# DaehwanKimLab/tophat

Hardware: AMD Instinct MI355X
Metric: paired reads/sec through segment_juncs+long_spanning_reads; junctions.bed diff=0 (higher is better)
Workload: dtype u64

## Files before the change

### tophat_amd/csrc/thj_core.h

```cpp
#pragma once
#include <stdint.h>

#if defined(__HIPCC__)
#define THJ_HD __host__ __device__ __forceinline__
#else
#define THJ_HD inline
#endif

#if defined(THJ_EXP) && defined(__HIPCC__)
static __device__ int thj_exp_flags;
#define THJ_EXPF(b) (thj_exp_flags & (b))
#else
#define THJ_EXPF(b) 0
#endif

namespace thj {

typedef unsigned long long u64;

THJ_HD int popc(u64 x) { return __builtin_popcountll(x); }
THJ_HD int popc32(uint32_t x) { return __builtin_popcount(x); }
THJ_HD int ctz(u64 x) { return __builtin_ctzll(x); }
THJ_HD int clz(u64 x) { return __builtin_clzll(x); }
THJ_HD u64 lowmask(int n) { return n >= 64 ? ~0ull : ((1ull << n) - 1ull); }
// ... 564 lines not shown
template <int NS>
THJ_HD bool read_is_trivial_flat(const Params& p, const ReadView& v) {
    const int nseg = v.nseg;
    const uint32_t first = v.so[0];
    if (v.so[nseg] == first) return true;
    bool single = true;
#pragma unroll
    for (int s = 0; s < NS; ++s) single = single && (s >= nseg || v.so[s + 1] - v.so[s] == 1u);
    if (!single) return false;
    Hit h[NS];
#pragma unroll
    for (int s = 0; s < NS; ++s) if (s < nseg) h[s] = v.hits[first + s];
    const Hit h0 = h[0];
    const bool anti = hit_anti(h0);
    if (nseg == 1) return hit_end(h0) || v.n_mate == 0;
    const int L = p.segment_length;
    bool ok = true;
    Hit prev = h0;
#pragma unroll
    for (int s = 1; s < NS; ++s) {
        if (s < nseg) {
            const Hit c = h[s];
            ok = ok && c.ref_id == h0.ref_id && hit_anti(c) == anti;
            ok = ok && (anti ? c.right == prev.left : prev.right == c.left);
            if (s + 1 < nseg) {
                const int start = (s - 1) * L;
                const int plen = v.rl - start < 2 * L ? v.rl - start : 2 * L;
                const int apparent = anti ? prev.right - c.left : c.right - prev.left;
                ok = ok && start <= v.rl && apparent == plen;
            }
            prev = c;
        }
    }
    if (!ok) return false;
    const int dist = anti ? h0.left - prev.right : prev.left - h0.right;
    if (dist >= p.min_segment_intron && dist < p.max_segment_intron) return true;
    return v.n_mate == 0;
}

THJ_HD bool read_is_trivial(const Params& p, const ReadView& v) {
    if (v.nseg < 1) return true;
    if (v.nseg <= 4) return read_is_trivial_flat<4>(p, v);
    const uint32_t first = v.so[0];
    if (v.so[v.nseg] == first) return true;
    for (int s = 0; s < v.nseg; ++s) if (v.so[s + 1] - v.so[s] != 1u) return false;
    const Hit h0 = v.hits[first];
    const bool anti = hit_anti(h0);
    if (v.nseg == 1) return hit_end(h0) || v.n_mate == 0;
    const int L = p.segment_length;
    Hit prev = h0;
    for (int s = 1; s < v.nseg; ++s) {
        const Hit h = v.hits[first + s];
        if (h.ref_id != h0.ref_id || hit_anti(h) != anti) return false;
        if (!((anti && h.right == prev.left) || (!anti && prev.right == h.left))) return false;
        if (s + 1 < v.nseg) {
            const int start = (s - 1) * L;
            if (start > v.rl) return false;
            const int plen = v.rl - start < 2 * L ? v.rl - start : 2 * L;
            const int apparent = anti ? prev.right - h.left : h.right - prev.left;
            if (apparent != plen) return false;
        }
        prev = h;
    }
    const int dist = anti ? h0.left - prev.right : prev.left - h0.right;
    if (dist >= p.min_segment_intron && dist < p.max_segment_intron) return true;
    return v.n_mate == 0;
}

THJ_HD uint32_t task_window_word(bool anti, int start, int slen) { return (anti ? 1u << 9 : 0u) | ((uint32_t)(start & 511) << 10) | ((uint32_t)(slen & 127) << 19); }
THJ_HD uint32_t task_indel_word(bool anti, bool is_del, int i, int plen) {
    return (1u << 8) | (anti ? 1u << 9 : 0u) | (is_del ? 1u << 10 : 0u) | ((uint32_t)(i & 15) << 11) | ((uint32_t)(plen & 255) << 15);
}
THJ_HD bool task_is_indel(uint32_t a) { return (a & (1u << 8)) != 0; }
THJ_HD bool task_anti(uint32_t a) { return ((a >> 9) & 1u) != 0; }
THJ_HD bool task_is_del(uint32_t a) { return ((a >> 10) & 1u) != 0; }
THJ_HD int task_indel_i(uint32_t a) { return (int)((a >> 11) & 15u); }
THJ_HD int task_indel_plen(uint32_t a) { return (int)((a >> 15) & 255u); }
THJ_HD int task_window_start(uint32_t a) { return (int)((a >> 10) & 511u); }
THJ_HD int task_window_slen(uint32_t a) { return (int)((a >> 19) & 127u); }

struct FlatResult { bool rescue; int size; int n_windows, n_indels; };

template <int NS, class Emit>
THJ_HD FlatResult flat_read(const Params& p, int nseg, const uint32_t (&so)[NS + 1], const Hit (&h)[NS], int rl, int n_mate, Emit& emit) {
    FlatResult res{false, 0, 0, 0};
    const int L = p.segment_length;
    uint32_t present = 0;
#pragma unroll
    for (int s = 0; s < NS; ++s) if (s < nseg && so[s + 1] != so[s]) present |= 1u << s;
    bool go = true;
#pragma unroll
    for (int i = 0; i + 2 < NS; ++i) {
        const int start = i * L;
        go = go && i + 2 < nseg && ((present >> i) & 3u) == 3u && start <= rl;
        const int plen = rl - start < 2 * L ? rl - start : 2 * L;
        const Hit lh = h[i], rh = h[i + 1];
        const bool anti = hit_anti(lh);
        const int apparent = anti ? lh.right - rh.left : rh.right - lh.left;
        const int disc = apparent - plen;
        const bool is_del = disc > 0 && disc <= p.max_deletion_length;
        const bool is_ins = disc < 0 && disc >= -p.max_insertion_length;
        const bool ok = go && lh.ref_id == rh.ref_id && anti == hit_anti(rh) && (is_del || is_ins);
        emit.task(ok, task_indel_word(anti, is_del, i, plen), anti ? so[i + 1] : so[i], anti ? so[i] : so[i + 1], 0u);
        res.n_indels += ok ? 1 : 0;
    }
    int last = 0;
    Hit hl = h[0];
#pragma unroll
    for (int s = 1; s < NS; ++s) if ((present >> s) & 1u) { last = s; hl = h[s]; }
    res.size = last + 1;
    bool run = nseg > 0;
    if (last == 0) run = run && (present & 1u) && !hit_end(h[0]);
    bool check_partner = true;
    if (last != 0 && (present & 1u) && h[0].ref_id == hl.ref_id && hit_anti(h[0]) == hit_anti(hl)) {
        const int dist = hit_anti(h[0]) ? h[0].left - hl.right : hl.left - h[0].right;
        if (dist >= p.min_segment_intron && dist < p.max_segment_intron) check_partner = false;
    }
    res.rescue = run && check_partner && n_mate > 0;
    bool en = run && !res.rescue;
    if (p.bowtie2 && present != 0 && 1 > p.max_seg_multihits) en = false;
#pragma unroll
    for (int s = 0; s + 1 < NS; ++s) {
        const bool has = en && s != last && ((present >> s) & 1u);
        const Hit bh = h[s];
        const bool banti = hit_anti(bh);
        const Hit rh = h[s + 1];
        const bool c1 = ((present >> (s + 1)) & 1u) && banti == hit_anti(rh) && bh.ref_id == rh.ref_id;
        const bool abut = banti ? rh.right == bh.left : bh.right == rh.left;
        const int d1 = banti ? bh.left - rh.right : rh.left - bh.right;
        const bool found = c1 && abut;
        const bool drs = c1 && !abut && d1 >= p.min_segment_intron && d1 < p.max_segment_intron;
        bool rrs = false;
        Hit d = rh;
        if (s + 2 < NS) {
            const Hit rrh = h[s + 2];
            const bool c2 = ((present >> (s + 2)) & 1u) && banti == hit_anti(rrh) && bh.ref_id == rrh.ref_id;
            const int d2 = banti ? bh.left - rrh.right : rrh.left - bh.right;
            rrs = !found && c2 && d2 >= p.min_segment_intron + L && d2 < p.max_segment_intron + L;
            if (rrs) d = rrh;
        }
        const int start = (s + 1) * L - 8;
        int slen = rrs ? L + 16 : 16;
        if (slen > rl - start) slen = rl - start;
        int32_t wl, wr;
        if (!banti) { wl = bh.right - 8; if (wl < 0) wl = 0; wr = d.left + 8; }
        else { wl = d.right - 8; wr = bh.left + 8; }
        const bool ok = has && !found && (drs || rrs) && start >= 0 && slen >= 0;
        emit.task(ok, task_window_word(banti, start, slen), bh.ref_id, (uint32_t)wl, (uint32_t)wr);
        res.n_windows += ok ? 1 : 0;
    }
    return res;
}

enum { SLOT_UNSCANNED = -3 };
template <int MAXM, class Emit>
THJ_HD int flat_rescue(const Params& p, bool has0, const Hit& bh, int size, int rl, const Hit (&mh)[MAXM], int n_mate,
                       const int32_t (&sc)[2 * MAXM], Emit& emit, int& n_windows) {
    const int L = p.segment_length;
    int cl = L - p.segment_mismatches - 3;
    if (cl > 15) cl = 15;
    const bool banti = hit_anti(bh);
    bool alive = has0;
    int pairs = 0, n_pseudo = 0;
    int32_t pl[2 * MAXM];
    bool pv[2 * MAXM];
#pragma unroll
    for (int m = 0; m < MAXM; ++m) {
        const bool compat = alive && m < n_mate && bh.ref_id == mh[m].ref_id && banti != hit_anti(mh[m]);
        const int32_t f = compat ? sc[2 * m] : SLOT_NONE, rv = compat ? sc[2 * m + 1] : SLOT_NONE;
        if (compat && f == SLOT_BREAK) alive = false;
        pairs += (compat && f != SLOT_BREAK && f != SLOT_UNSCANNED) ? 1 : 0;
        pv[2 * m] = compat && alive && f >= 0; pl[2 * m] = f;
        pv[2 * m + 1] = compat && alive && rv >= 0; pl[2 * m + 1] = rv;
        n_pseudo += (pv[2 * m] ? 1 : 0) + (pv[2 * m + 1] ? 1 : 0);
    }
    bool en = has0 && (size == 2 || size == 3);
    if (p.bowtie2 && (1 > p.max_seg_multihits || n_pseudo > p.max_seg_multihits)) en = false;
    const bool far = size == 3;
    const int lo = p.min_segment_intron + (far ? L : 0), hi = p.max_segment_intron + (far ? L : 0);
    bool found = false, inr[2 * MAXM];
    int n = 0;
#pragma unroll
    for (int k = 0; k < 2 * MAXM; ++k) {
        const bool panti = (k & 1) != 0;
        const bool c = pv[k] && banti == panti;
        const int32_t pleft = pl[k], pright = pl[k] + cl;
        const bool abut = banti ? pright == bh.left : bh.right == pleft;
        if (c && abut && !far) found = true;
        const int dist = banti ? bh.left - pright : pleft - bh.right;
        inr[k] = c && dist >= lo && dist < hi;
        n += inr[k] ? 1 : 0;
    }
    const int start = L - 8;
    int slen = far ? L + 16 : 16;
    if (slen > rl - start) slen = rl - start;
    const bool ok_all = en && !found && n > 0 && start >= 0 && slen >= 0;
#pragma unroll
    for (int k = 0; k < 2 * MAXM; ++k) {
        const int32_t pleft = pl[k], pright = pl[k] + cl;
        int32_t wl, wr;
        if (!banti) { wl = bh.right - 8; if (wl < 0) wl = 0; wr = pleft + 8; }
        else { wl = pright - 8; wr = bh.left + 8; }
        const bool ok = ok_all && inr[k];
        emit.task(ok, task_window_word(banti, start, slen), bh.ref_id, (uint32_t)wl, (uint32_t)wr);
        n_windows += ok ? 1 : 0;
    }
    return pairs;
}

template <class Sink>
THJ_HD void gaps_enumerate(const Params& p, const ReadView& v, Sink& sink, int first = 0, int stride = 1) {
    const int L = p.segment_length;
    if (p.bowtie2)
        for (int s = 0; s < v.size; ++s) {
            int n = (!v.rescue || s == 0) ? rv_count_raw(v, s) : rv_count(v, s);
            if (n > p.max_seg_multihits) return;
        }
    for (int s = 0; s < v.size; ++s) {
        rv_foreach_strided(v, s, first, stride, [&](const Hit& bh) {
            bool found = (s == v.size - 1);
            int n_drs = 0, n_rrs = 0;
            const bool banti = hit_anti(bh);
            if (s < v.size - 1) {
                rv_foreach(v, s + 1, [&](const Hit& rh) {
                    if (banti != hit_anti(rh) || bh.ref_id != rh.ref_id) return true;
                    if ((banti && rh.right == bh.left) || (!banti && bh.right == rh.left)) { found = true; return false; }
                    int dist = banti ? bh.left - rh.right : rh.left - bh.right;
                    if (dist >= p.min_segment_intron && dist < p.max_segment_intron) ++n_drs;
                    return true;
                });
            }
            if (!found && s < v.size - 2) {
                rv_foreach(v, s + 2, [&](const Hit& rrh) {
                    if (banti != hit_anti(rrh) || bh.ref_id != rrh.ref_id) return true;
                    int dist = banti ? bh.left - rrh.right : rrh.left - bh.right;
                    if (dist >= p.min_segment_intron + L && dist < p.max_segment_intron + L) ++n_rrs;
                    return true;
                });
            }
            if (!found && (n_drs > 0 || n_rrs > 0)) {
                const bool use_rrs = n_rrs > 0;
                const int lo = p.min_segment_intron + (use_rrs ? L : 0);
                const int hi = p.max_segment_intron + (use_rrs ? L : 0);
                const int start = (s + 1) * L - 8;
                int slen = use_rrs ? L + 16 : 16;
                if (slen > v.rl - start) slen = v.rl - start;
                if (start >= 0 && slen >= 0) {
                    rv_foreach(v, use_rrs ? s + 2 : s + 1, [&](const Hit& d) {
                        if (banti != hit_anti(d) || bh.ref_id != d.ref_id) return true;
                        int dist = banti ? bh.left - d.right : d.left - bh.right;
                        if (dist < lo || dist >= hi) return true;
                        int32_t wl, wr;
                        if (!banti) { wl = bh.right - 8; if (wl < 0) wl = 0; wr = d.left + 8; }
                        else { wl = d.right - 8; wr = bh.left + 8; }
                        sink.window(bh.ref_id, wl, wr, banti, start, slen);
                        return true;
                    });
                }
            }
        });
    }
}

template <class X>
THJ_HD Hit wave_bcast_hit(X& x, const Hit& h, int src) {
    Hit o;
    o.ref_id = x.bcast(h.ref_id, src); o.left = (int32_t)x.bcast((uint32_t)h.left, src);
    o.right = (int32_t)x.bcast((uint32_t)h.right, src); o.meta = x.bcast(h.meta, src);
    return o;
}
THJ_HD Hit wave_lane_hit(const ReadView& v, int s, int lane) {
    Hit h{0, 0, 0, 0};
    if (lane < rv_count_raw(v, s)) h = v.hits[v.so[s] + (uint32_t)lane];
    return h;
}
THJ_HD bool wave_read_fits(const ReadView& v) {
    for (int s = 0; s < v.nseg; ++s) if (rv_count_raw(v, s) > 64) return false;
    return true;
}
template <class X, class Sink>
THJ_HD bool wave_read_enumerate(X& x, const Params& p, ReadView& v, Sink& sink, bool& wants_rescue) {
    const int lane = x.lane;
    const int L = p.segment_length;
    wants_rescue = false;
    v.rescue = false;
    v.check_len = p.segment_length - p.segment_mismatches - 3;
    if (v.check_len > 15) v.check_len = 15;
    if (v.nseg == 0) return false;
    int last = v.nseg - 1;
    while (last > 0 && rv_count_raw(v, last) == 0) --last;
    v.size = last + 1;
    if (last == 0) {
        if (rv_count_raw(v, 0) == 0) return false;
        const Hit h0 = v.hits[v.so[0]];
        if (hit_end(h0)) return false;
    }
    {
        bool found = false;
        if (last != 0) {
            const Hit lh = wave_lane_hit(v, 0, lane);
            const bool have = lane < rv_count_raw(v, 0);
            const Hit D = wave_lane_hit(v, last, lane);
            const int nD = rv_count_raw(v, last);
            for (int j = 0; j < nD; ++j) {
                const Hit rh = wave_bcast_hit(x, D, j);
                if (have && lh.ref_id == rh.ref_id && hit_anti(lh) == hit_anti(rh)) {
// ... 351 lines not shown
```

### tophat_amd/csrc/thj_segjuncs.hip

```cpp
#include <hip/hip_runtime.h>
#include <hipcub/hipcub.hpp>

#include <cstdio>
#include <cstdlib>
#include <algorithm>
#include <cstring>
#include <cstddef>
#include <chrono>
#include <vector>

#include "../../include/thj.h"
#include "thj_core.h"
#include "thj_fusion_block.h"
#include "thj_internal.h"

using namespace thj;

static_assert(sizeof(thj_hit) == 16 && sizeof(Hit) == 16, "hit layout");
static_assert(sizeof(thj_params) == sizeof(Params), "params layout");




static constexpr u64 EMPTY = ~0ull;
// ... 3 lines not shown
struct Tables {
    u64* junc; u64 junc_mask;
    u64* del;  u64 del_mask;
    u64* ins_key; u64* ins_val; u64 ins_mask;
    u64* junc_list; u64* del_list; u64* ins_list;
    unsigned int* ovf;
    unsigned long long* cnt;
};

__device__ __forceinline__ u64 mix64(u64 x) {
    x ^= x >> 30; x *= 0xbf58476d1ce4e5b9ull;
    x ^= x >> 27; x *= 0x94d049bb133111ebull;
    x ^= x >> 31;
    return x;
}

__device__ __forceinline__ unsigned long long list_append_pos(unsigned long long* count) {
    const int lane = (int)(threadIdx.x & 63u);
    const unsigned long long below = lane ? (~0ull >> (64 - lane)) : 0ull;
    for (;;) {
        const unsigned long long mine_p = (unsigned long long)count;
        const unsigned long long p0 = ((unsigned long long)(uint32_t)__builtin_amdgcn_readfirstlane((int)(uint32_t)(mine_p >> 32)) << 32) |
                                      (uint32_t)__builtin_amdgcn_readfirstlane((int)(uint32_t)mine_p);
        const bool now = mine_p == p0;
        const unsigned long long grp = __ballot(now);
        if (now) {
            unsigned long long base = 0;
            if (lane == __ffsll((long long)grp) - 1) base = atomicAdd(count, (unsigned long long)__popcll(grp));
            const uint32_t lo = (uint32_t)__builtin_amdgcn_readfirstlane((int)(uint32_t)base), hi = (uint32_t)__builtin_amdgcn_readfirstlane((int)(uint32_t)(base >> 32));
            return (((unsigned long long)hi << 32) | lo) + (unsigned long long)__popcll(grp & below);
        }
    }
}

static constexpr u64 PROBE_CAP = 4096;
template <bool RESCUE = false>
__device__ __forceinline__ void set_insert(u64* tab, u64 mask, u64 key, unsigned long long* count, unsigned int* ovf, u64* list) {
    if (!RESCUE && __hip_atomic_load(ovf, __ATOMIC_RELAXED, __HIP_MEMORY_SCOPE_AGENT) != 0u) return;
    u64 h = mix64(key) & mask;
    const u64 limit = RESCUE ? mask : (mask < PROBE_CAP ? mask : PROBE_CAP);
    for (u64 probe = 0; probe <= limit; ++probe) {
        u64 cur = __hip_atomic_load(&tab[h], __ATOMIC_RELAXED, __HIP_MEMORY_SCOPE_AGENT);
        if (cur == key) return;
        if (cur == EMPTY) {
            u64 old = atomicCAS((unsigned long long*)&tab[h], EMPTY, key);
            if (old == EMPTY) { const unsigned long long pos = list_append_pos(count); if (pos <= mask) list[pos] = key; return; }
            if (old == key) return;
        }
        h = (h + 1) & mask;
    }
    atomicExch(ovf, 1u);
}

template <bool RESCUE = false>
__device__ __forceinline__ void map_insert_min(u64* keys, u64* vals, u64 mask, u64 key, u64 val,
                                               unsigned long long* count, unsigned int* ovf, u64* list) {
    if (!RESCUE && __hip_atomic_load(ovf, __ATOMIC_RELAXED, __HIP_MEMORY_SCOPE_AGENT) != 0u) return;
    u64 h = mix64(key) & mask;
    const u64 limit = RESCUE ? mask : (mask < PROBE_CAP ? mask : PROBE_CAP);
    for (u64 probe = 0; probe <= limit; ++probe) {
        u64 cur = __hip_atomic_load(&keys[h], __ATOMIC_RELAXED, __HIP_MEMORY_SCOPE_AGENT);
        if (cur == EMPTY) {
            u64 old = atomicCAS((unsigned long long*)&keys[h], EMPTY, key);
            if (old == EMPTY) { const unsigned long long pos = list_append_pos(count); if (pos <= mask) list[pos] = h; cur = key; }
            else cur = old;
        }
        if (cur == key) { atomicMin((unsigned long long*)&vals[h], val); return; }
        h = (h + 1) & mask;
    }
    atomicExch(ovf, 1u);
}

struct EventSink {
    const Genome& g;
    const Tables& t;
    __device__ __forceinline__ void junction(uint32_t ref, uint32_t l, uint32_t r, bool a) {
        set_insert(t.junc, t.junc_mask, junc_key(g, ref, l, r, a), &t.cnt[CNT_JUNC], &t.ovf[0], t.junc_list);
    }
    __device__ __forceinline__ void deletion(uint32_t ref, uint32_t l, uint32_t r) {
        set_insert(t.del, t.del_mask, junc_key(g, ref, l, r, false), &t.cnt[CNT_DEL], &t.ovf[1], t.del_list);
    }
    __device__ __forceinline__ void insertion(uint32_t ref, uint32_t l, int len, uint32_t seq, u64 prio) {
        map_insert_min(t.ins_key, t.ins_val, t.ins_mask, ins_key(g, ref, l, len), (prio << INS_SEQ_BITS) | (u64)(seq & ((1u << INS_SEQ_BITS) - 1u)),
                       &t.cnt[CNT_INS], &t.ovf[2], t.ins_list);
    }
};


struct DevBatch {
    int32_t n_reads, nseg, W, pad;
    const uint32_t* seg_off;
    const Hit* hits;
    const u64* planes;
    const uint16_t* read_len;
    const uint32_t* mate_off;
    const Hit* mate_hits;
    uint32_t ordinal_base, pad2;
};
static_assert(sizeof(DevBatch) == sizeof(thj_seg_batch), "batch layout");

__device__ __forceinline__ ReadView make_view(const DevBatch& b, int r) {
    ReadView v;
    v.hits = b.hits;
    v.so = b.seg_off + (size_t)r * b.nseg;
    v.nseg = b.nseg;
    v.W = b.W;
    v.rp = b.planes + (size_t)r * 3 * b.W;
    v.rl = b.read_len[r];
    v.mate = nullptr; v.n_mate = 0; v.slots = nullptr; v.mscan = nullptr;
    if (b.mate_off) {
        uint32_t m0 = b.mate_off[r], m1 = b.mate_off[r + 1];
        v.mate = b.mate_hits + m0;
        v.n_mate = (int)(m1 - m0);
    }
    v.size = 0; v.rescue = false; v.check_len = 0;
    return v;
}


static constexpr int TPB = 256;
static constexpr int QCAP = 512;
static constexpr int MANY_CAP = 1 << 20;
static constexpr int MANY_HITS_LDS = 256;

struct Queue {
    uint32_t* a; uint32_t* b; uint32_t* c; uint32_t* d; uint32_t* e;
    unsigned int* n;
};
struct XTasks { uint4* q; uint32_t* e; unsigned int* count; unsigned int cap; unsigned int* ovf; };

struct QueueSink {
    Queue q;
    XTasks x;
    uint32_t read;
    uint32_t hbase;
    unsigned int n_windows, n_indels;
    __device__ __forceinline__ void push(uint32_t a, uint32_t b, uint32_t c, uint32_t d) {
        unsigned int k = atomicAdd(q.n, 1u);
        if (k < (unsigned)QCAP) { q.a[k] = a; q.b[k] = b; q.c[k] = c; q.d[k] = d; q.e[k] = read; }
        else {
            const unsigned int pos = atomicAdd(x.count, 1u);
            if (pos < x.cap) { x.q[pos] = make_uint4(a, b, c, d); x.e[pos] = read; } else atomicExch(x.ovf, 1u);
        }
    }
    __device__ __forceinline__ void window(uint32_t ref, int32_t wl, int32_t wr, bool anti, int start, int slen) {
        ++n_windows;
        push(task_window_word(anti, start, slen), ref, (uint32_t)wl, (uint32_t)wr);
    }
    __device__ __forceinline__ void indel(int i, uint32_t lidx, uint32_t ridx, int li, int ri, bool anti, int plen, bool is_del) {
        ++n_indels;
        push(task_indel_word(anti, is_del, i, plen), lidx + hbase, ridx + hbase, (uint32_t)li | ((uint32_t)ri << 16));
    }
};
__device__ __forceinline__ void flush_tasks(const Queue& q, const XTasks& x, unsigned int* s_base, unsigned int* full_rounds) {
    __syncthreads();
    const unsigned int have = *q.n, n = have < (unsigned)QCAP ? have : (unsigned)QCAP;
    if (have == 0) return;
    if (threadIdx.x == 0) { *s_base = atomicAdd(x.count, n); if (have > (unsigned)QCAP) atomicAdd(full_rounds, 1u); }
    __syncthreads();
    const unsigned int base = *s_base;
    for (unsigned int k = threadIdx.x; k < n; k += blockDim.x) {
        const unsigned int pos = base + k;
        if (pos < x.cap) { x.q[pos] = make_uint4(q.a[k], q.b[k], q.c[k], q.d[k]); x.e[pos] = q.e[k]; } else atomicExch(x.ovf, 1u);
    }
    __syncthreads();
    if (threadIdx.x == 0) *q.n = 0;
}

__device__ __forceinline__ ReadView make_task_view(const DevBatch& b, int r) {
    ReadView v;
    v.hits = b.hits;
    v.so = b.seg_off + (size_t)r * b.nseg;
    v.nseg = b.nseg;
    v.W = b.W;
    v.rp = b.planes + (size_t)r * 3 * b.W;
    v.rl = b.read_len[r];
    v.mate = nullptr; v.n_mate = 0; v.slots = nullptr; v.mscan = nullptr;
    v.size = 0; v.rescue = false; v.check_len = 0;
    return v;
}

struct RescueList { uint32_t* list; unsigned int* blk_cnt; int seg_cap; int32_t* slot_pool; unsigned int* heavy_count; uint32_t* heavy_list;
                    unsigned int* many_count; uint32_t* many_list; int own_slice; int many_min; int mid_min; };

struct SjLists {
    uint4* tq; uint32_t* te; unsigned int* task_cnt; int task_cap;
    uint32_t* frl; unsigned int* frl_cnt;
    uint32_t* pairs; unsigned int* pair_cnt;
    int2* scan;
    uint32_t* gen; unsigned int* gen_cnt;
    unsigned int* mid_count; uint32_t* mid_list;
};
static constexpr int FLAT_MATES = 2;
static constexpr uint32_t GEN_READ = (1u << 29) - 1;

struct FlatEmit {
    uint4* tq; uint32_t* te; unsigned int* n; unsigned long long below; uint32_t read;
    __device__ __forceinline__ void task(bool ok, uint32_t a, uint32_t b, uint32_t c, uint32_t d) {
        const unsigned long long m = __ballot(ok);
        if (m == 0) return;
        unsigned int base = 0;
        if ((threadIdx.x & 63) == 0) base = atomicAdd(n, (unsigned int)__popcll(m));
        base = (unsigned int)__shfl((int)base, 0);
        if (ok) { const unsigned int k = base + (unsigned int)__popcll(m & below); tq[k] = make_uint4(a, b, c, d); te[k] = read; }
    }
};
__device__ __forceinline__ unsigned int wave_slot(bool want, unsigned int* counter, unsigned long long below) {
    const unsigned long long m = __ballot(want);
    if (m == 0) return 0u;
    unsigned int base = 0;
    if ((threadIdx.x & 63) == 0) base = atomicAdd(counter, (unsigned int)__popcll(m));
    base = (unsigned int)__shfl((int)base, 0);
    return base + (unsigned int)__popcll(m & below);
}

template <int NS>
__global__ __launch_bounds__(TPB, 4) void thj_k_sj_flat(Params p, DevBatch b, RescueList rl, SjLists sl, unsigned long long* cnt) {
    __shared__ unsigned int s_n[4];
    __shared__ unsigned int s_stat[3];
    const int tid = threadIdx.x, lane = tid & 63;
    if (tid < 4) s_n[tid] = 0;
    if (tid < 3) s_stat[tid] = 0;
    __syncthreads();
    const unsigned long long below = lane ? (~0ull >> (64 - lane)) : 0ull;
    const size_t slice = (size_t)blockIdx.x * rl.seg_cap;
    uint4* const tq = sl.tq + (size_t)blockIdx.x * sl.task_cap;
    uint32_t* const te = sl.te + (size_t)blockIdx.x * sl.task_cap;
    const int nseg = b.nseg;
    unsigned int my_hits = 0, my_windows = 0, my_indels = 0;
    const int n_tiles = (b.n_reads + TPB - 1) / TPB;
    for (int tile = blockIdx.x; tile < n_tiles; tile += gridDim.x) {
        const int r = tile * TPB + tid;
        const bool active = r < b.n_reads;
        uint32_t so[NS + 1];
#pragma unroll
        for (int k = 0; k <= NS; ++k) so[k] = 0;
        if (active) {
            const uint32_t* o = b.seg_off + (size_t)r * nseg;
            if (NS == 4 && nseg == 4) { const uint4 q = *(const uint4*)o; so[0] = q.x; so[1] = q.y; so[2] = q.z; so[3] = q.w; so[4] = o[4]; }
            else {
#pragma unroll
                for (int k = 0; k <= NS; ++k) so[k] = o[k <= nseg ? k : nseg];
            }
        }
        const uint32_t nh = so[NS] - so[0];
        int n_mate = 0;
        if (active && b.mate_off) n_mate = (int)(b.mate_off[r + 1] - b.mate_off[r]);
        bool single = n_mate <= FLAT_MATES;
#pragma unroll
        for (int s = 0; s < NS; ++s) single = single && so[s + 1] - so[s] <= 1u;
        my_hits += nh;
        const bool is_flat = active && single && nh > 0;
        {
            const bool gen = active && !single;
            const unsigned int gk = wave_slot(gen, &s_n[3], below);
            if (gen) sl.gen[slice + gk] = (uint32_t)r | (nh > (uint32_t)rl.many_min ? 2u << 29 : nh > (uint32_t)rl.mid_min ? 1u << 29 : 0u);
        }
        Hit h[NS];
#pragma unroll
        for (int s = 0; s < NS; ++s) {
            uint4 q = make_uint4(0, 0, 0, 0);
            if (is_flat && so[s + 1] != so[s]) q = ((const uint4*)b.hits)[so[s]];
            h[s].ref_id = q.x; h[s].left = (int32_t)q.y; h[s].right = (int32_t)q.z; h[s].meta = q.w;
        }
        int rlen = 0;
        if (is_flat) rlen = b.read_len[r];
        FlatEmit em{tq, te, &s_n[0], below, (uint32_t)r};
        const FlatResult res = flat_read<NS>(p, is_flat ? nseg : 0, so, h, rlen, n_mate, em);
        my_windows += (unsigned int)res.n_windows; my_indels += (unsigned int)res.n_indels;
        const bool resc_flat = res.rescue && so[1] != so[0];
        const unsigned int fk = wave_slot(resc_flat, &s_n[1], below);
        if (resc_flat) sl.frl[slice + fk] = (uint32_t)r | ((uint32_t)(res.size - 1 < 7 ? res.size - 1 : 7) << 29);
#pragma unroll
        for (int m = 0; m < FLAT_MATES; ++m) {
            const bool want = resc_flat && m < n_mate;
            const unsigned int pk = wave_slot(want, &s_n[2], below);
            if (want) sl.pairs[slice * FLAT_MATES + pk] = (fk << 1) | (uint32_t)m;
        }
    }
    if (my_hits) atomicAdd(&s_stat[2], my_hits);
    if (my_windows) atomicAdd(&s_stat[0], my_windows);
    if (my_indels) atomicAdd(&s_stat[1], my_indels);
    __syncthreads();
    {
        __shared__ unsigned int s_nlist[2], s_lbase[2];
        const unsigned int n_gen = s_n[3];
        for (unsigned int k0 = 0; k0 < n_gen; k0 += TPB) {
            const unsigned int k = k0 + (unsigned int)tid;
            const uint32_t e = k < n_gen ? sl.gen[slice + k] : 0u;
            const bool mid = (e >> 29) == 1u, many = (e >> 29) == 2u;
            if (tid < 2) s_nlist[tid] = 0;
            __syncthreads();
            const unsigned int dk = wave_slot(mid, &s_nlist[0], below), mk = wave_slot(many, &s_nlist[1], below);
            __syncthreads();
            if (tid == 0 && s_nlist[0]) s_lbase[0] = atomicAdd(sl.mid_count, s_nlist[0]);
            if (tid == 64 && s_nlist[1]) s_lbase[1] = atomicAdd(rl.many_count, s_nlist[1]);
            __syncthreads();
            if (mid) { if (s_lbase[0] + dk < (unsigned int)MANY_CAP) sl.mid_list[s_lbase[0] + dk] = e & GEN_READ; else sl.gen[slice + k] = e & GEN_READ; }
            if (many) { if (s_lbase[1] + mk < (unsigned int)MANY_CAP) rl.many_list[s_lbase[1] + mk] = e & GEN_READ; else sl.gen[slice + k] = e & GEN_READ; }
        }
    }
    if (tid == 0) {
        sl.task_cnt[blockIdx.x] = s_n[0]; sl.frl_cnt[blockIdx.x] = s_n[1]; sl.pair_cnt[blockIdx.x] = s_n[2]; sl.gen_cnt[blockIdx.x] = s_n[3];
        rl.blk_cnt[blockIdx.x] = 0;
        if (s_stat[0]) atomicAdd(&cnt[CNT_WINDOWS], (unsigned long long)s_stat[0]);
        if (s_stat[1]) atomicAdd(&cnt[CNT_INDEL_PAIRS], (unsigned long long)s_stat[1]);
        if (s_stat[2]) atomicAdd(&cnt[CNT_HITS], (unsigned long long)s_stat[2]);
    }
}

template <bool WIDE>
__device__ __forceinline__ void exec_task(const Genome& g, const Params& p, const DevBatch& b, EventSink& ev, const uint4 q, const int tr) {
    ReadView tv = make_task_view(b, tr);
    const uint32_t a = q.x;
    const bool anti = task_anti(a);
    if (task_is_indel(a)) {
        const int i = task_indel_i(a);
        indel_exec<WIDE>(g, p, tv, i, q.y, q.z, anti, task_indel_plen(a), task_is_del(a),
                   ins_prio(b.ordinal_base + (uint32_t)tr, i, (int)(q.w & 0xFFFF), (int)(q.w >> 16)), ev);
    } else
        window_exec<WIDE>(g, p, tv, q.y, (int32_t)q.z, (int32_t)q.w, anti, task_window_start(a), task_window_slen(a), ev);
}
static constexpr int TASK_DEFER_CAP = 3072;
template <bool WIDE>
__global__ __launch_bounds__(TPB) void thj_k_sj_tasks(Genome g, Params p, DevBatch b, Tables t, SjLists sl) {
    __shared__ uint32_t s_defer[TASK_DEFER_CAP];
    __shared__ unsigned int s_nd;
    const unsigned int n = sl.task_cnt[blockIdx.x];
    const uint4* tq = sl.tq + (size_t)blockIdx.x * sl.task_cap;
    const uint32_t* te = sl.te + (size_t)blockIdx.x * sl.task_cap;
    const int lane = (int)(threadIdx.x & 63u);
    const unsigned long long below = lane ? (~0ull >> (64 - lane)) : 0ull;
    if (threadIdx.x == 0) s_nd = 0;
    __syncthreads();
    EventSink ev{g, t};
    for (unsigned int k0 = 0; k0 < n; k0 += TPB) {
        const unsigned int k = k0 + threadIdx.x;
        const bool active = k < n;
        uint4 q = make_uint4(0, 0, 0, 0);
        if (active) q = tq[k];
        const bool indel = active && task_is_indel(q.x);
        const unsigned int slot = wave_slot(indel, &s_nd, below);
        if (indel && slot < (unsigned int)TASK_DEFER_CAP) s_defer[slot] = k;
        else if (active) exec_task<WIDE>(g, p, b, ev, q, (int)te[k]);
    }
    __syncthreads();
    const unsigned int nd = s_nd < (unsigned int)TASK_DEFER_CAP ? s_nd : (unsigned int)TASK_DEFER_CAP;
    for (unsigned int j = threadIdx.x; j < nd; j += TPB) {
        const unsigned int k = s_defer[j];
        const uint4 q = tq[k];
        const int tr = (int)te[k];
        ReadView tv = make_task_view(b, tr);
        const int i = task_indel_i(q.x);
        indel_exec<WIDE>(g, p, tv, i, q.y, q.z, task_anti(q.x), task_indel_plen(q.x), task_is_del(q.x),
                         ins_prio(b.ordinal_base + (uint32_t)tr, i, (int)(q.w & 0xFFFF), (int)(q.w >> 16)), ev);
    }
}
template <bool WIDE>
__global__ __launch_bounds__(TPB) void thj_k_sj_tasks_list(Genome g, Params p, DevBatch b, Tables t, XTasks x) {
    const unsigned int n = *x.count < x.cap ? *x.count : x.cap;
    EventSink ev{g, t};
    for (unsigned int k = blockIdx.x * TPB + threadIdx.x; k < n; k += gridDim.x * TPB) exec_task<WIDE>(g, p, b, ev, x.q[k], (int)x.e[k]);
}

__global__ __launch_bounds__(TPB) void thj_k_sj_rescue_scan(Genome g, Params p, DevBatch b, SjLists sl, int seg_cap) {
    const unsigned int n = sl.pair_cnt[blockIdx.x];
    const size_t slice = (size_t)blockIdx.x * seg_cap;
    for (unsigned int k = threadIdx.x; k < n; k += TPB) {
        const uint32_t e = sl.pairs[slice * FLAT_MATES + k];
        const uint32_t slot = e >> 1, m = e & 1u;
        const int r = (int)(sl.frl[slice + slot] & 0x1FFFFFFFu);
        const uint4 q = ((const uint4*)b.mate_hits)[b.mate_off[r] + m];
        Hit rh; rh.ref_id = q.x; rh.left = (int32_t)q.y; rh.right = (int32_t)q.z; rh.meta = q.w;
        int32_t f, rv;
        const bool scanned = rescue_scan(g, p, b.planes + (size_t)r * 3 * b.W, b.W, (int)b.read_len[r], rh, f, rv);
        if (!scanned && f != SLOT_BREAK) f = SLOT_UNSCANNED;
        sl.scan[(slice + slot) * FLAT_MATES + m] = make_int2(f, rv);
    }
}

__global__ __launch_bounds__(TPB) void thj_k_sj_rescue_flat(Params p, DevBatch b, SjLists sl, int seg_cap, unsigned long long* cnt, unsigned int* n_flat_pairs) {
    __shared__ unsigned int s_ntask, s_stat[2];
    const int tid = threadIdx.x, lane = tid & 63;
    const unsigned int n = sl.frl_cnt[blockIdx.x];
    if (tid == 0) { s_ntask = sl.task_cnt[blockIdx.x]; s_stat[0] = 0; s_stat[1] = 0; }
    __syncthreads();
    const unsigned long long below = lane ? (~0ull >> (64 - lane)) : 0ull;
    const size_t slice = (size_t)blockIdx.x * seg_cap;
    unsigned int my_pairs = 0, my_windows = 0;
    for (unsigned int k0 = 0; k0 < n; k0 += TPB) {
        const unsigned int k = k0 + (unsigned int)tid;
        const bool active = k < n;
        int r = 0, size = 0, n_mate = 0, rlen = 0;
        Hit bh{0, 0, 0, 0}, mh[FLAT_MATES];
        int32_t sc[2 * FLAT_MATES];
#pragma unroll
        for (int m = 0; m < FLAT_MATES; ++m) { mh[m] = Hit{0, 0, 0, 0}; sc[2 * m] = SLOT_NONE; sc[2 * m + 1] = SLOT_NONE; }
        if (active) {
            const uint32_t e = sl.frl[slice + k];
            r = (int)(e & 0x1FFFFFFFu); size = (int)(e >> 29) + 1;
            const uint4 q = ((const uint4*)b.hits)[b.seg_off[(size_t)r * b.nseg]];
            bh.ref_id = q.x; bh.left = (int32_t)q.y; bh.right = (int32_t)q.z; bh.meta = q.w;
            rlen = b.read_len[r];
            const uint32_t m0 = b.mate_off[r];
            n_mate = (int)(b.mate_off[r + 1] - m0);
#pragma unroll
            for (int m = 0; m < FLAT_MATES; ++m)
                if (m < n_mate) {
                    const uint4 w = ((const uint4*)b.mate_hits)[m0 + m];
                    mh[m].ref_id = w.x; mh[m].left = (int32_t)w.y; mh[m].right = (int32_t)w.z; mh[m].meta = w.w;
                    const int2 o = sl.scan[(slice + k) * FLAT_MATES + m];
                    sc[2 * m] = o.x; sc[2 * m + 1] = o.y;
                }
        }
        FlatEmit em{sl.tq + (size_t)blockIdx.x * sl.task_cap, sl.te + (size_t)blockIdx.x * sl.task_cap, &s_ntask, below, (uint32_t)r};
        int nw = 0;
        my_pairs += (unsigned int)flat_rescue<FLAT_MATES>(p, active, bh, size, rlen, mh, n_mate, sc, em, nw);
        my_windows += (unsigned int)nw;
    }
    if (my_pairs) atomicAdd(&s_stat[0], my_pairs);
    if (my_windows) atomicAdd(&s_stat[1], my_windows);
    __syncthreads();
    if (tid == 0) {
        sl.task_cnt[blockIdx.x] = s_ntask;
        if (s_stat[0]) { atomicAdd(&cnt[CNT_RESCUE_PAIRS], (unsigned long long)s_stat[0]); atomicAdd(n_flat_pairs, s_stat[0]); }
        if (s_stat[1]) atomicAdd(&cnt[CNT_WINDOWS], (unsigned long long)s_stat[1]);
    }
}

#ifndef THJ_GEN_HITS
#define THJ_GEN_HITS 8
#endif
static constexpr int GEN_HITS = THJ_GEN_HITS;
static constexpr int MID_HITS = 32;
static constexpr int MID_T = 256;
static constexpr int MID_G = 8;
static constexpr int MID_GRID = 2048;
#ifndef THJ_GEN_G
#define THJ_GEN_G 4
#endif
static constexpr int GEN_G = THJ_GEN_G;
template <int HITS, int T, bool SLICED, int SO, int G = 1>
__global__ __launch_bounds__(T) void thj_k_sj_general(Params p, DevBatch b, RescueList rl, SjLists sl, XTasks x, unsigned long long* cnt) {
    static_assert(G >= 1 && G <= 64 && (G & (G - 1)) == 0 && T % G == 0, "lanes per read");
    constexpr int RPR = T / G;
    constexpr int STRIDE = HITS + 1;
    __shared__ uint32_t q_a[QCAP], q_b[QCAP], q_c[QCAP], q_d[QCAP], q_e[QCAP];
    __shared__ uint4 s_hits[RPR * STRIDE];
    __shared__ uint32_t s_so[RPR * SO];
    __shared__ unsigned int q_n, s_nresc, s_base[3], s_xbase;
    __shared__ unsigned int s_stat[4];
    const int tid = threadIdx.x, lane = tid & 63, slot = tid / G, g = tid % G;
    if (tid < 4) s_stat[tid] = 0;
    if (tid == 0) { q_n = 0; s_nresc = 0; }
    __syncthreads();
    const unsigned long long below = lane ? (~0ull >> (64 - lane)) : 0ull;
    const Queue qq{q_a, q_b, q_c, q_d, q_e, &q_n};
    const unsigned int n = SLICED ? sl.gen_cnt[blockIdx.x] : (*sl.mid_count < (unsigned int)MANY_CAP ? *sl.mid_count : (unsigned int)MANY_CAP);
    const uint32_t* list = SLICED ? sl.gen + (size_t)blockIdx.x * rl.seg_cap : sl.mid_list;
    const unsigned int first = SLICED ? 0u : blockIdx.x * RPR, step = SLICED ? (unsigned int)RPR : gridDim.x * RPR;
    unsigned int my_windows = 0, my_indels = 0;
    for (unsigned int k0 = first; k0 < n; k0 += step) {
        __syncthreads();
        const unsigned int k = k0 + (unsigned int)slot;
        bool active = k < n;
        ReadView v;
        bool do_gaps = false, to_rescue = false;
        int r = 0;
        uint32_t hbase = 0;
        const uint32_t e = active ? list[k] : 0u;
        r = (int)(e & GEN_READ);
        if (SLICED && (e >> 29) != 0u) active = false;
        if (active) {
            v = make_view(b, r);
            const uint32_t h0 = v.so[0], nh = v.so[v.nseg] - h0;
            if (nh <= (uint32_t)HITS) {
                for (int i = g; i <= v.nseg; i += G) s_so[slot * SO + i] = v.so[i] - h0;
                for (uint32_t i = (uint32_t)g; i < nh; i += (uint32_t)G) s_hits[slot * STRIDE + i] = ((const uint4*)b.hits)[h0 + i];
                v.so = s_so + slot * SO; v.hits = (const Hit*)(s_hits + slot * STRIDE); hbase = h0;
            }
        }
        __builtin_amdgcn_fence(__ATOMIC_RELEASE, "wavefront"); __builtin_amdgcn_wave_barrier(); __builtin_amdgcn_fence(__ATOMIC_ACQUIRE, "wavefront");
        if (active) {
            bool wants = false;
            if (G == 1) do_gaps = !THJ_EXPF(1 << 18) && gaps_prepare(p, v, wants);
            else do_gaps = !THJ_EXPF(1 << 18) && gaps_prepare_shared(p, v, wants, g, G, [&](bool f) { return ((__ballot(f) >> (lane - g)) & (~0ull >> (64 - G))) != 0ull; });
            to_rescue = do_gaps && wants;
            if (!to_rescue) {
                QueueSink qs{qq, x, (uint32_t)r, hbase, 0u, 0u};
                if (!THJ_EXPF(1 << 17)) indels_enumerate(p, v, qs, g, G);
                if (do_gaps) gaps_enumerate(p, v, qs, g, G);
                my_windows += qs.n_windows; my_indels += qs.n_indels;
            }
        }
        const bool resc = to_rescue && g == 0;
        if (SLICED) {
            const unsigned int rk = wave_slot(resc, &s_nresc, below);
            if (resc) rl.list[(size_t)blockIdx.x * rl.seg_cap + rk] = (uint32_t)r;
        } else {
            if (tid == 0) s_nresc = 0;
            __syncthreads();
            const unsigned int rk = wave_slot(resc, &s_nresc, below);
            __syncthreads();
            if (tid == 0 && s_nresc) s_base[2] = atomicAdd(&rl.blk_cnt[rl.own_slice], s_nresc);
            __syncthreads();
            if (resc) rl.list[(size_t)rl.own_slice * rl.seg_cap + s_base[2] + rk] = (uint32_t)r;
        }
        flush_tasks(qq, x, &s_xbase, &s_stat[3]);
    }
    if (my_windows) atomicAdd(&s_stat[0], my_windows);
    if (my_indels) atomicAdd(&s_stat[1], my_indels);
    __syncthreads();
    if (tid == 0) {
        if (SLICED) rl.blk_cnt[blockIdx.x] = s_nresc;
        if (s_stat[0]) atomicAdd(&cnt[CNT_WINDOWS], (unsigned long long)s_stat[0]);
        if (s_stat[1]) atomicAdd(&cnt[CNT_INDEL_PAIRS], (unsigned long long)s_stat[1]);
        if (s_stat[3]) atomicAdd(&cnt[CNT_OVF_BLOCKS], (unsigned long long)s_stat[3]);
    }
}

struct SjWave {
    int lane;
    __device__ __forceinline__ unsigned long long ballot(bool p) { return __ballot(p); }
    __device__ __forceinline__ uint32_t bcast(uint32_t v, int src) { return (uint32_t)__builtin_amdgcn_readlane((int)v, __builtin_amdgcn_readfirstlane(src)); }
};
__global__ __launch_bounds__(TPB, 4) void thj_k_segjuncs_shared(Params p, DevBatch b, RescueList rl, XTasks x, unsigned long long* cnt) {
    __shared__ uint32_t q_a[QCAP], q_b[QCAP], q_c[QCAP], q_d[QCAP], q_e[QCAP];
    __shared__ unsigned int q_n;
    __shared__ unsigned int s_stat[4];
    __shared__ Hit s_h[TPB / 64][MANY_HITS_LDS];
    __shared__ uint32_t s_o[TPB / 64][20];
    const int tid = threadIdx.x, lane = tid & 63, wave = tid >> 6;
    if (tid < 4) s_stat[tid] = 0;
    if (tid == 0) q_n = 0;
    __syncthreads();
    const Queue qq{q_a, q_b, q_c, q_d, q_e, &q_n};
    const unsigned int n = *rl.many_count < (unsigned int)MANY_CAP ? *rl.many_count : (unsigned int)MANY_CAP;
    const unsigned int SHARED_BATCH = n / gridDim.x >= 32u ? 32u : n / gridDim.x >= 4u ? n / gridDim.x : 4u;
    __shared__ unsigned int s_next, s_batch, s_nr, s_rbase, s_xbase;
    __shared__ uint32_t s_resc[32];
    if (tid == 0) s_nr = 0;
    unsigned int my_windows = 0, my_indels = 0;
    for (;;) {
        __syncthreads();
        if (tid == 0) { s_next = 0; s_batch = atomicAdd(rl.many_count + 1, 1u); }
        __syncthreads();
        const unsigned int base = s_batch * SHARED_BATCH;
        if (base >= n) break;
        for (;;) {
            unsigned int k = 0;
            if (lane == 0) k = atomicAdd(&s_next, 1u);
            k = (unsigned int)__shfl((int)k, 0);
            if (k >= SHARED_BATCH || base + k >= n) break;
            const int r = (int)rl.many_list[base + k];
            ReadView v = make_view(b, r);
            bool do_gaps = false, wants = false, staged = false;
            uint32_t hbase = 0;
            const uint32_t h0 = v.so[0], nh = v.so[v.nseg] - h0;
            __builtin_amdgcn_fence(__ATOMIC_RELEASE, "wavefront"); __builtin_amdgcn_wave_barrier(); __builtin_amdgcn_fence(__ATOMIC_ACQUIRE, "wavefront");
            if (nh <= (uint32_t)MANY_HITS_LDS && v.nseg < 20) {
                for (uint32_t i = (uint32_t)lane; i < nh; i += 64u) ((uint4*)s_h[wave])[i] = ((const uint4*)b.hits)[h0 + i];
                if (lane <= v.nseg) s_o[wave][lane] = v.so[lane] - h0;
                __builtin_amdgcn_fence(__ATOMIC_RELEASE, "wavefront"); __builtin_amdgcn_wave_barrier(); __builtin_amdgcn_fence(__ATOMIC_ACQUIRE, "wavefront");
                v.hits = s_h[wave]; v.so = s_o[wave]; hbase = h0; staged = true;
            }
            if (THJ_EXPF(1 << 26)) continue;
            if (staged && wave_read_fits(v)) {
                SjWave xw{lane};
                QueueSink qs{qq, x, (uint32_t)r, hbase, 0u, 0u};
                do_gaps = wave_read_enumerate(xw, p, v, qs, wants);
                if (do_gaps && wants) { if (lane == 0) s_resc[atomicAdd(&s_nr, 1u)] = (uint32_t)r; }
                else { my_windows += qs.n_windows; my_indels += qs.n_indels; }
                continue;
            }
            do_gaps = gaps_prepare_shared(p, v, wants, lane, 64, [](bool f) { return __any((int)f) != 0; });
            if (THJ_EXPF(1 << 27)) continue;
            if (do_gaps && wants) {
                if (lane == 0) s_resc[atomicAdd(&s_nr, 1u)] = (uint32_t)r;
            } else {
                QueueSink qs{qq, x, (uint32_t)r, hbase, 0u, 0u};
                if (!THJ_EXPF(1 << 17)) indels_enumerate(p, v, qs, lane, 64);
                if (do_gaps && !THJ_EXPF(1 << 25)) gaps_enumerate(p, v, qs, lane, 64);
                my_windows += qs.n_windows; my_indels += qs.n_indels;
            }
        }
        __syncthreads();
        if (s_nr) {
            if (tid == 0) s_rbase = atomicAdd(&rl.blk_cnt[rl.own_slice], s_nr);
            __syncthreads();
            if ((unsigned int)tid < s_nr) rl.list[(size_t)rl.own_slice * rl.seg_cap + s_rbase + tid] = s_resc[tid];
            __syncthreads();
            if (tid == 0) s_nr = 0;
        }
        flush_tasks(qq, x, &s_xbase, &s_stat[3]);
    }
    if (my_windows) atomicAdd(&s_stat[0], my_windows);
    if (my_indels) atomicAdd(&s_stat[1], my_indels);
    __syncthreads();
    if (tid == 0) {
        if (s_stat[0]) atomicAdd(&cnt[CNT_WINDOWS], (unsigned long long)s_stat[0]);
        if (s_stat[1]) atomicAdd(&cnt[CNT_INDEL_PAIRS], (unsigned long long)s_stat[1]);
        if (s_stat[3]) atomicAdd(&cnt[CNT_OVF_BLOCKS], (unsigned long long)s_stat[3]);
    }
}

static constexpr int RPT = 4;
static constexpr int MSCAN = 128;
static constexpr int RESCUE_GRID = 1024;
static constexpr int HEAVY_CAP = 1 << 18;
static constexpr int MAX_LISTS = 2048;

__global__ __launch_bounds__(TPB, 4) void thj_k_segjuncs_rescue(Genome g, Params p, DevBatch b, RescueList rl, int n_lists, XTasks x, unsigned long long* cnt) {
    __shared__ uint32_t q_a[QCAP], q_b[QCAP], q_c[QCAP], q_d[QCAP], q_e[QCAP];
    __shared__ int32_t s_slots[TPB * RPT * 2];
    __shared__ unsigned int s_off[MAX_LISTS + 1];
    __shared__ unsigned int q_n;
    __shared__ unsigned int s_stat[4];
    __shared__ Genome s_g;
    __shared__ Params s_p;
    typedef hipcub::BlockScan<unsigned int, TPB> Scan;
    __shared__ typename Scan::TempStorage scan_tmp;
    __shared__ unsigned int s_nheavy, s_heavy_base, s_xbase;
    const int tid = threadIdx.x;
    const unsigned long long below = (tid & 63) ? (~0ull >> (64 - (tid & 63))) : 0ull;
    if (tid < 4) s_stat[tid] = 0;
    if (tid == 0) { q_n = 0; s_g = g; s_p = p; }
    unsigned int total;
    {
        constexpr int IPT = MAX_LISTS / TPB;
        unsigned int cnt[IPT], sum = 0, excl;
#pragma unroll
        for (int k = 0; k < IPT; ++k) { const int j = tid * IPT + k; cnt[k] = j < n_lists ? rl.blk_cnt[j] : 0u; sum += cnt[k]; }
        Scan(scan_tmp).ExclusiveSum(sum, excl, total);
#pragma unroll
        for (int k = 0; k < IPT; ++k) { s_off[tid * IPT + k] = excl; excl += cnt[k]; }
        if (tid == 0) s_off[MAX_LISTS] = total;
    }
    __syncthreads();
    const Queue qq{q_a, q_b, q_c, q_d, q_e, &q_n};
    const unsigned int per_round = gridDim.x * TPB;
    const unsigned int rounds = (total + per_round - 1) / per_round;
    unsigned int my_pairs = 0, my_windows = 0, my_indels = 0;
    for (unsigned int it = 0; it < rounds; ++it) {
        const unsigned int i = (it * gridDim.x + blockIdx.x) * TPB + tid;
        const bool active = i < total;
        __syncthreads();
        ReadView v;
        bool do_gaps = false, heavy = false;
        int r = 0;
        if (active) {
            int lo = 0, hi = n_lists;
            while (hi - lo > 1) { const int mid = (lo + hi) >> 1; if (s_off[mid] <= i) lo = mid; else hi = mid; }
            r = (int)rl.list[(size_t)lo * rl.seg_cap + (i - s_off[lo])];
            v = make_view(b, r);
            heavy = (int64_t)rv_count_raw(v, 0) * v.n_mate > RPT && v.n_mate <= MSCAN && !THJ_EXPF(1 << 24);
        }
        unsigned int hk = 0;
        {
            if (tid == 0) s_nheavy = 0;
            __syncthreads();
            hk = wave_slot(heavy, &s_nheavy, below);
// ... 1263 lines not shown
```

Baseline: 2.077 billion.

## Pre-screen two-hit-per-segment general reads with a flat per-thread pass

Reads whose segments each have at most two hits are tagged during classification. In the sliced general kernel they are first evaluated with a new per-thread flat2_read routine that only detects whether any task or rescue would be produced. Reads that emit nothing are dropped, and rescues are recorded directly. The remaining reads are compacted into shared memory before the cooperative general rounds run, which avoids spending group rounds on empty reads. The cost is an extra pass with duplicated per-thread logic, which risks divergence from the general path's semantics.

```diff
diff --git a/tophat_amd/csrc/thj_core.h b/tophat_amd/csrc/thj_core.h
--- a/tophat_amd/csrc/thj_core.h
+++ b/tophat_amd/csrc/thj_core.h
@@ -740,6 +740,113 @@
     return res;
 }
 
+template <int NS, class Emit>
+THJ_HD FlatResult flat2_read(const Params& p, int nseg, const uint32_t (&so)[NS + 1], const uint32_t (&n)[NS], const Hit (&h)[NS][2], int rl, int n_mate, Emit& emit) {
+    FlatResult res{false, 0, 0, 0};
+    const int L = p.segment_length;
+    uint32_t cn[NS];
+#pragma unroll
+    for (int s = 0; s < NS; ++s) cn[s] = s < nseg ? n[s] : 0u;
+    uint32_t key[NS][2];
+    int32_t lo[NS][2], hi[NS][2];
+#pragma unroll
+    for (int s = 0; s < NS; ++s)
+#pragma unroll
+        for (int a = 0; a < 2; ++a) {
+            const bool anti = hit_anti(h[s][a]);
+            key[s][a] = (h[s][a].ref_id << 1) | (anti ? 1u : 0u);
+            lo[s][a] = anti ? -h[s][a].right : h[s][a].left;
+            hi[s][a] = anti ? -h[s][a].left : h[s][a].right;
+        }
+    int last = 0;
+#pragma unroll
+    for (int s = 1; s < NS; ++s) if (cn[s] != 0u) last = s;
+    res.size = last + 1;
+    bool run = nseg > 0;
+    if (last == 0) run = run && cn[0] != 0u && !hit_end(h[0][0]);
+    bool partner = false;
+#pragma unroll
+    for (int s = 1; s < NS; ++s)
+#pragma unroll
+        for (int a = 0; a < 2; ++a)
+#pragma unroll
+            for (int b = 0; b < 2; ++b) {
+                const int dist = lo[s][b] - hi[0][a];
+                partner = partner || (last == s && (uint32_t)a < cn[0] && (uint32_t)b < cn[s] && key[0][a] == key[s][b] &&
+                                      dist >= p.min_segment_intron && dist < p.max_segment_intron);
+            }
+    res.rescue = run && !partner && n_mate > 0;
+    bool go = !res.rescue;
+#pragma unroll
+    for (int i = 0; i + 2 < NS; ++i) {
+        const int start = i * L;
+        go = go && i + 2 < nseg && cn[i] != 0u && cn[i + 1] != 0u && start <= rl;
+        const int plen = rl - start < 2 * L ? rl - start : 2 * L;
+#pragma unroll
+        for (int a = 0; a < 2; ++a)
+#pragma unroll
+            for (int b = 0; b < 2; ++b) {
+                const bool anti = (key[i][a] & 1u) != 0;
+                const int disc = hi[i + 1][b] - lo[i][a] - plen;
+                const bool is_del = disc > 0 && disc <= p.max_deletion_length;
+                const bool is_ins = disc < 0 && disc >= -p.max_insertion_length;
+                const bool ok = go && (uint32_t)a < cn[i] && (uint32_t)b < cn[i + 1] && key[i][a] == key[i + 1][b] && (is_del || is_ins);
+                const uint32_t li = so[i] + (uint32_t)a, ri = so[i + 1] + (uint32_t)b;
+                emit.task(ok, task_indel_word(anti, is_del, i, plen), anti ? ri : li, anti ? li : ri, (uint32_t)a | ((uint32_t)b << 16));
+                res.n_indels += ok ? 1 : 0;
+            }
+    }
+    bool en = run && !res.rescue;
+#pragma unroll
+    for (int s = 0; s < NS; ++s) if (p.bowtie2 && s <= last && (int)cn[s] > p.max_seg_multihits) en = false;
+#pragma unroll
+    for (int s = 0; s + 1 < NS; ++s)
+#pragma unroll
+        for (int a = 0; a < 2; ++a) {
+            const bool has = en && s < last && (uint32_t)a < cn[s];
+            const uint32_t bkey = key[s][a];
+            const int32_t bhi = hi[s][a];
+            const bool banti = (bkey & 1u) != 0;
+            bool found = false, drs = false, rrs = false;
+            bool in1[2], in2[2] = {false, false};
+#pragma unroll
+            for (int b = 0; b < 2; ++b) {
+                const bool c1 = (uint32_t)b < cn[s + 1] && bkey == key[s + 1][b];
+                const int d1 = lo[s + 1][b] - bhi;
+                found = found || (c1 && d1 == 0);
+                in1[b] = c1 && d1 != 0 && d1 >= p.min_segment_intron && d1 < p.max_segment_intron;
+                drs = drs || in1[b];
+            }
+            if (s + 2 < NS) {
+#pragma unroll
+                for (int b = 0; b < 2; ++b) {
+                    const bool c2 = (uint32_t)b < cn[s + 2] && bkey == key[s + 2][b];
+                    const int d2 = lo[s + 2][b] - bhi;
+                    in2[b] = c2 && d2 >= p.min_segment_intron + L && d2 < p.max_segment_intron + L;
+                    rrs = rrs || in2[b];
+                }
+            }
+            const int start = (s + 1) * L - 8;
+            const bool emits = has && !found && (drs || rrs) && start >= 0 && (rrs ? L + 16 : 16) >= 0 && rl - start >= 0;
+#pragma unroll
+            for (int b = 0; b < 2; ++b) {
+                bool in = in1[b];
+                if (s + 2 < NS) in = rrs ? in2[b] : in;
+                const bool ok = emits && in;
+                int slen = rrs ? L + 16 : 16;
+                if (slen > rl - start) slen = rl - start;
+                int32_t dlo = lo[s + 1][b];
+                if (s + 2 < NS) dlo = rrs ? lo[s + 2][b] : dlo;
+                int32_t wl, wr;
+                if (!banti) { wl = bhi - 8; if (wl < 0) wl = 0; wr = dlo + 8; }
+                else { wl = -dlo - 8; wr = -bhi + 8; }
+                emit.task(ok, task_window_word(banti, start, slen), bkey >> 1, (uint32_t)wl, (uint32_t)wr);
+                res.n_windows += ok ? 1 : 0;
+            }
+        }
+    return res;
+}
+
 enum { SLOT_UNSCANNED = -3 };
 template <int MAXM, class Emit>
 THJ_HD int flat_rescue(const Params& p, bool has0, const Hit& bh, int size, int rl, const Hit (&mh)[MAXM], int n_mate,
diff --git a/tophat_amd/csrc/thj_segjuncs.hip b/tophat_amd/csrc/thj_segjuncs.hip
--- a/tophat_amd/csrc/thj_segjuncs.hip
+++ b/tophat_amd/csrc/thj_segjuncs.hip
@@ -179,6 +179,10 @@
         push(task_indel_word(anti, is_del, i, plen), lidx + hbase, ridx + hbase, (uint32_t)li | ((uint32_t)ri << 16));
     }
 };
+struct AnyTask {
+    bool any;
+    __device__ __forceinline__ void task(bool ok, uint32_t, uint32_t, uint32_t, uint32_t) { any = any || ok; }
+};
 __device__ __forceinline__ void flush_tasks(const Queue& q, const XTasks& x, unsigned int* s_base, unsigned int* full_rounds) {
     __syncthreads();
     const unsigned int have = *q.n, n = have < (unsigned)QCAP ? have : (unsigned)QCAP;
@@ -220,6 +224,7 @@
 };
 static constexpr int FLAT_MATES = 2;
 static constexpr uint32_t GEN_READ = (1u << 29) - 1;
+static constexpr uint32_t GEN_TWO = 3u;
 
 struct FlatEmit {
     uint4* tq; uint32_t* te; unsigned int* n; unsigned long long below; uint32_t read;
@@ -280,8 +285,11 @@
         const bool is_flat = active && single && nh > 0;
         {
             const bool gen = active && !single;
+            bool two = NS == 4;
+#pragma unroll
+            for (int s = 0; s < NS; ++s) two = two && so[s + 1] - so[s] <= 2u;
             const unsigned int gk = wave_slot(gen, &s_n[3], below);
-            if (gen) sl.gen[slice + gk] = (uint32_t)r | (nh > (uint32_t)rl.many_min ? 2u << 29 : nh > (uint32_t)rl.mid_min ? 1u << 29 : 0u);
+            if (gen) sl.gen[slice + gk] = (uint32_t)r | (nh > (uint32_t)rl.many_min ? 2u << 29 : nh > (uint32_t)rl.mid_min ? 1u << 29 : two ? GEN_TWO << 29 : 0u);
         }
         Hit h[NS];
 #pragma unroll
@@ -487,17 +495,11 @@
     const uint32_t* list = SLICED ? sl.gen + (size_t)blockIdx.x * rl.seg_cap : sl.mid_list;
     const unsigned int first = SLICED ? 0u : blockIdx.x * RPR, step = SLICED ? (unsigned int)RPR : gridDim.x * RPR;
     unsigned int my_windows = 0, my_indels = 0;
-    for (unsigned int k0 = first; k0 < n; k0 += step) {
+    auto general_round = [&](bool active, const int r) {
         __syncthreads();
-        const unsigned int k = k0 + (unsigned int)slot;
-        bool active = k < n;
         ReadView v;
         bool do_gaps = false, to_rescue = false;
-        int r = 0;
         uint32_t hbase = 0;
-        const uint32_t e = active ? list[k] : 0u;
-        r = (int)(e & GEN_READ);
-        if (SLICED && (e >> 29) != 0u) active = false;
         if (active) {
             v = make_view(b, r);
             const uint32_t h0 = v.so[0], nh = v.so[v.nseg] - h0;
@@ -534,6 +536,72 @@
             if (resc) rl.list[(size_t)rl.own_slice * rl.seg_cap + s_base[2] + rk] = (uint32_t)r;
         }
         flush_tasks(qq, x, &s_xbase, &s_stat[3]);
+    };
+    if constexpr (SLICED) {
+        uint32_t* const gen = sl.gen + (size_t)blockIdx.x * rl.seg_cap;
+        if constexpr (SO == 9) {
+            if (b.nseg <= 4)
+                for (unsigned int k0 = 0; k0 < n; k0 += (unsigned int)T) {
+                    const unsigned int k = k0 + (unsigned int)tid;
+                    const uint32_t e = k < n ? gen[k] : 0u;
+                    const bool two = k < n && (e >> 29) == GEN_TWO;
+                    const int r = (int)(e & GEN_READ);
+                    const int nseg = b.nseg;
+                    uint32_t so[5] = {0u, 0u, 0u, 0u, 0u}, cn[4], m0 = 0, m1 = 0;
+                    int rlen = 0;
+                    if (two) {
+                        const uint32_t* o = b.seg_off + (size_t)r * nseg;
+                        if (nseg == 4) { const uint4 q = *(const uint4*)o; so[0] = q.x; so[1] = q.y; so[2] = q.z; so[3] = q.w; so[4] = o[4]; }
+                        else {
+#pragma unroll
+                            for (int i = 0; i <= 4; ++i) so[i] = o[i <= nseg ? i : nseg];
+                        }
+                        rlen = b.read_len[r];
+                        if (b.mate_off) { m0 = b.mate_off[r]; m1 = b.mate_off[r + 1]; }
+                    }
+                    THJ_LOADS_ISSUED();
+                    Hit h[4][2];
+#pragma unroll
+                    for (int s = 0; s < 4; ++s) {
+                        cn[s] = so[s + 1] - so[s];
+#pragma unroll
+                        for (int a = 0; a < 2; ++a) {
+                            uint4 q = make_uint4(0, 0, 0, 0);
+                            if (two && (uint32_t)a < cn[s]) q = ((const uint4*)b.hits)[so[s] + (uint32_t)a];
+                            h[s][a].ref_id = q.x; h[s][a].left = (int32_t)q.y; h[s][a].right = (int32_t)q.z; h[s][a].meta = q.w;
+                        }
+                    }
+                    THJ_LOADS_ISSUED();
+                    AnyTask at{false};
+                    const FlatResult res = flat2_read<4>(p, two ? nseg : 0, so, cn, h, rlen, (int)(m1 - m0), at);
+                    if (at.any) gen[k] = (uint32_t)r;
+                    const unsigned int rk = wave_slot(res.rescue, &s_nresc, below);
+                    if (res.rescue) rl.list[(size_t)blockIdx.x * rl.seg_cap + rk] = (uint32_t)r;
+                }
+        }
+        __shared__ uint32_t s_pick[T];
+        __shared__ unsigned int s_npick;
+        for (unsigned int k0 = 0; k0 < n; k0 += (unsigned int)T) {
+            __syncthreads();
+            if (tid == 0) s_npick = 0;
+            __syncthreads();
+            const unsigned int k = k0 + (unsigned int)tid;
+            const uint32_t e = k < n ? gen[k] : 0u;
+            const bool mine = k < n && (e >> 29) == 0u;
+            const unsigned int pk = wave_slot(mine, &s_npick, below);
+            if (mine) s_pick[pk] = e;
+            __syncthreads();
+            const unsigned int np = s_npick;
+            for (unsigned int j0 = 0; j0 < np; j0 += (unsigned int)RPR) {
+                const unsigned int j = j0 + (unsigned int)slot;
+                general_round(j < np, j < np ? (int)s_pick[j] : 0);
+            }
+        }
+    } else {
+        for (unsigned int k0 = first; k0 < n; k0 += step) {
+            const unsigned int k = k0 + (unsigned int)slot;
+            general_round(k < n, k < n ? (int)(list[k] & GEN_READ) : 0);
+        }
     }
     if (my_windows) atomicAdd(&s_stat[0], my_windows);
     if (my_indels) atomicAdd(&s_stat[1], my_indels);
```

Result: faster. 2.113 billion, median of 6 (+1.7%).
